# yaki-toki/5G-NR-RandomAccess

Measured on AMD Instinct MI355X. Metric: UE-subframe updates/sec at nUE=100k Beta; bit-exact success-ratio vs ref, higher is better.
Workload: dtype int32

## Files before the change

### 5g-nr-randomaccess_amd/csrc/prach_device.h

```cpp
#pragma once
#include <hip/hip_runtime.h>
#include <stdint.h>
#include "../../include/prach.h"

namespace prach {

constexpr unsigned PK_ACT_SHIFT = 0, PK_CONN_SHIFT = 2, PK_PRE_SHIFT = 4, PK_RAR_SHIFT = 12, PK_MRC_SHIFT = 20,
                   PK_PEND_SHIFT = 28;
constexpr int ACT_IDLE = 0;
constexpr int ACT_DONE = 1;
constexpr int ACT_M1 = 2;
constexpr int ACT_M3 = 3;

constexpr int PEND_NONE = 0, PEND_STAY = 1, PEND_CALLER = 2, PEND_RESET = 3, PEND_PASSIVE = 4, PEND_RJOIN = 5;
constexpr unsigned PK_GRANT_BIT = 0x80000000u;
constexpr int EV_CALLER = 1, EV_RESETCAND = 2, EV_PASSIVE = 3, EV_RJOIN = 4;

struct alignas(16) Event {
    int idx;
    int info;
    int le;
    int pad;
};

// ... 73 lines not shown
size_t trial_kernel_lds_bytes(int nP);
hipError_t launch_trial_kernel(const TrialDev *params, int ntrials, int rng_mode, int maxP, hipStream_t stream);
size_t cluster_kernel_lds_bytes(int nP, bool glibc, int lslots);
constexpr int CLUSTER_REC_G16 = 0, CLUSTER_REC_H8 = 1, CLUSTER_REC_L16 = 2;
constexpr int CLUSTER_EVW = 512;
constexpr int CLUSTER_REC_LFAST = 3;
size_t lcluster_kernel_lds_bytes(int lslots, bool glibc = false, int groups = 0);
int lcluster_group_capacity(int groups);
int lcluster_max_groups_glibc();
int lcluster_max_preambles();
hipError_t launch_lcluster_kernel(const TrialDev *params, int ntrials, int G, int lslots, int xpack, bool glibc, int groups, hipStream_t stream);
constexpr int CLUSTER_LQCAP = 4096;
constexpr size_t CLUSTER_LDS_LIMIT = 160 * 1024;
hipError_t launch_cluster_kernel(const TrialDev *params, int ntrials, int G, int maxP, int rng_mode, int rec_mode, int lslots, int xpack, hipStream_t stream);
int cluster_kernel_blocks_per_cu(int maxP, int rng_mode, int rec_mode, int lslots);
constexpr int CLUSTER_REC_BATCH = 4;
size_t batch_kernel_lds_bytes(int waves, bool glibc = false);
int batch_max_preambles();
int batch_max_rar_window();
int batch_max_subframes();
int batch_max_groups(bool glibc = false);
int batch_max_rar_window_two_per_cu();
int batch_chunk_bytes();
int batch_calendar_slots(int backoff, int accessTime, int maxRarWindow);
int batch_max_calendar_slots();
hipError_t launch_batch_kernel(const TrialDev *params, int ntrials, int waves, bool glibc, hipStream_t stream);
constexpr int STREAM_CHUNK = 31 * 2048;
hipError_t launch_glibc_stream(const unsigned *seeds, int *out, unsigned long long n, hipStream_t stream);
struct StreamJob { const unsigned *seeds; int *out; unsigned long long n; };
hipError_t launch_glibc_stream_jobs(const StreamJob *jobs, int njobs, unsigned long long max_n, hipStream_t stream);
extern "C" void prach_internal_glibc_seeds(uint32_t seed, uint64_t first, uint64_t nchunks, uint64_t chunk, uint32_t *out);
constexpr int CLUSTER_GLIBC_MAX_UE = 4096 * 64;
constexpr int CLUSTER_MAX_G = 64;
size_t noma_kernel_lds_bytes(int nP);
hipError_t launch_noma_kernel(const TrialDev *params, int ntrials, int G, int maxP, int xpack, hipStream_t stream);
int noma_kernel_blocks_per_cu(int maxP);
constexpr int NOMA_ACT_FLAG_CAP = 8192;
constexpr int NOMA_AMBIGUOUS = 77;
hipError_t launch_noma_activation(const TrialDev *params, int ntrials, int maxUE, unsigned *flags, hipStream_t stream);
constexpr int NOMA_GLIBC_AMBIGUOUS_RC = -1077;
int run_noma_glibc_trial(hipStream_t stream, const prach_cfg &c, const int32_t *hstream, unsigned long long len, prach_result *res, prach_ue_log *logs,
                         double *kernel_ms);
int run_noma_glibc_batch(hipStream_t stream, const prach_cfg *const *cfgs, int n, const unsigned long long *lens, prach_result *const *res, prach_ue_log *const *logs,
                         double *kernel_ms, int *rcs);

}
```

### 5g-nr-randomaccess_amd/csrc/prach_device_fn.h

```cpp
#pragma once
#include "prach_device.h"

#define PRACH_HD __host__ __device__ __forceinline__

namespace prach {

PRACH_HD int slot_align(int sub, int aT) {
    const int m = sub % aT;
    return m == 0 ? sub + 1 : (m == 1 ? sub : sub + (aT - m + 1));
}
struct FastMod { unsigned d, M; };
PRACH_HD unsigned mulhi32(const unsigned a, const unsigned b) { return (unsigned)(((unsigned long long)a * b) >> 32); }
PRACH_HD FastMod make_fastmod(int d) {
    FastMod f;
    f.d = (unsigned)d;
    f.M = d > 1 ? (unsigned)(0x100000000ull / (unsigned long long)d) : (d == 1 ? 0xFFFFFFFFu : 0u);
    return f;
}
PRACH_HD int fastmod(int x, const FastMod f) {
    if (f.d == 1u) return 0;
    const unsigned q = mulhi32((unsigned)x, f.M);
    const unsigned r = (unsigned)x - q * f.d;
    return (int)(r >= f.d ? r - f.d : r);
}
// ... 113 lines not shown
          n_lgain((const PRACH_G double *)d.n_lgain), n_nd0((const PRACH_G unsigned *)d.n_nd0), n_devact(d.n_devact), flags(d.flags), sector((PRACH_G int *)d.sector) {}
};

__device__ __forceinline__ int4 load_rec(const PRACH_G v4i_t *p) {
    const v4i_t v = __builtin_nontemporal_load(p);
    return make_int4(v.x, v.y, v.z, v.w);
}
__device__ __forceinline__ int4 load_rec_plain(const PRACH_G v4i_t *p) {
    const v4i_t v = *p;
    return make_int4(v.x, v.y, v.z, v.w);
}
__device__ __forceinline__ void store_rec(PRACH_G v4i_t *p, const int4 r) {
    v4i_t v;
    v.x = r.x; v.y = r.y; v.z = r.z; v.w = r.w;
    *p = v;
}
__device__ __forceinline__ void grant_rec(PRACH_G v4i_t *p) {
    __hip_atomic_fetch_or(reinterpret_cast<PRACH_G unsigned *>(p) + 3, PK_GRANT_BIT, __ATOMIC_RELAXED, __HIP_MEMORY_SCOPE_AGENT);
}
__device__ __forceinline__ void store_i2(PRACH_G v2i_t *p, const int a, const int b) {
    v2i_t v;
    v.x = a; v.y = b;
    *p = v;
}
__device__ __forceinline__ void store_log(PRACH_G v4i_t *logs, const int i, const prach_ue_log &o) {
    const int *w = reinterpret_cast<const int *>(&o);
#pragma unroll
    for (int k = 0; k < 4; k++) {
        v4i_t v;
        v.x = w[4 * k]; v.y = w[4 * k + 1]; v.z = w[4 * k + 2]; v.w = w[4 * k + 3];
        logs[(size_t)i * 4 + k] = v;
    }
}
struct PassMasks { unsigned long long light, quiet, done, trig; };
template <bool SPEC>
__device__ __forceinline__ PassMasks pass_masks(const unsigned pk, const int rx, const int rz, const int t, const unsigned rarlim, const bool front,
                                                const int i, const int acNow, const int acPrev, const int nUE) {
    typedef unsigned long long u64;
    const unsigned top = pk & 0xF0000000u;
    const u64 mM1 = __ballot((pk & 3u) == (unsigned)ACT_M1), mPre = __ballot((pk & (0xffu << PK_PRE_SHIFT)) != 0u);
    const u64 mBo = __ballot(rz <= t);
    const u64 mTrig = __ballot(rx == t);
    const u64 mPg0 = __ballot(pk < (1u << PK_PEND_SHIFT)), mAct2 = __ballot((pk & 2u) != 0u);
    u64 mDone = __ballot((pk & 3u) == (unsigned)ACT_DONE);
    const u64 mCont = mM1 & mPre & mBo;
    const unsigned age = top == ((unsigned)PEND_STAY << PK_PEND_SHIFT) ? (unsigned)(t - 1 - rx) : 0u;
    const unsigned rarnow = (pk & (0xffu << PK_RAR_SHIFT)) + (age << PK_RAR_SHIFT);
    u64 mLight = __ballot(pk < (3u << PK_PEND_SHIFT)) & mCont & __ballot(rarnow < rarlim);
    if (SPEC) mLight &= ~__ballot(top == ((unsigned)PEND_CALLER << PK_PEND_SHIFT));
    u64 mQuiet = mPg0 & (~mAct2 | (~mCont & ~mTrig & ~(mM1 & ~mPre)));
    if (front) {
        const u64 mValid = __ballot(i < acNow), mOld = __ballot(i < acPrev);
        mLight &= mOld;
        mQuiet = ~mValid | (mOld & mQuiet);
        mDone = (mValid & mDone) | __ballot(i >= nUE);
    }
    return PassMasks{mLight, mQuiet, mDone, mTrig};
}
__device__ __forceinline__ bool light_case(const unsigned pk, const int rx, const int rz, const int t, const unsigned rarlim) {
    const unsigned pg = pk >> PK_PEND_SHIFT;
    const bool contend = (pk & 3u) == (unsigned)ACT_M1 && (pk & (0xffu << PK_PRE_SHIFT)) != 0u && rz <= t;
    const int age = pg == (unsigned)PEND_STAY ? t - 1 - rx : 0;
    const unsigned rarnow = (pk & (0xffu << PK_RAR_SHIFT)) + ((unsigned)age << PK_RAR_SHIFT);
    return pg < 3u && contend && rarnow < rarlim;
}

template <class T> __device__ __forceinline__ void gadd(PRACH_G T *p, const T v) { __hip_atomic_fetch_add(p, v, __ATOMIC_RELAXED, __HIP_MEMORY_SCOPE_AGENT); }
template <class T> __device__ __forceinline__ void gmin(PRACH_G T *p, const T v) { __hip_atomic_fetch_min(p, v, __ATOMIC_RELAXED, __HIP_MEMORY_SCOPE_AGENT); }
template <class T> __device__ __forceinline__ void gmax(PRACH_G T *p, const T v) { __hip_atomic_fetch_max(p, v, __ATOMIC_RELAXED, __HIP_MEMORY_SCOPE_AGENT); }

struct UeState {
    int tx, tb, bo, act, conn, pre, rar, mrc, pend;
};
PRACH_HD UeState unpack(const int4 r) {
    UeState u;
    u.tx = r.x; u.tb = r.y; u.bo = r.z;
    u.act = (r.w >> PK_ACT_SHIFT) & 3; u.conn = (r.w >> PK_CONN_SHIFT) & 3; u.pre = (r.w >> PK_PRE_SHIFT) & 0xff;
    u.rar = (r.w >> PK_RAR_SHIFT) & 0xff; u.mrc = (r.w >> PK_MRC_SHIFT) & 0xff; u.pend = (r.w >> PK_PEND_SHIFT) & 7;
    return u;
}
PRACH_HD int4 pack(const UeState &u) {
    return make_int4(u.tx, u.tb, u.bo,
                     (u.act << PK_ACT_SHIFT) | (u.conn << PK_CONN_SHIFT) | (u.pre << PK_PRE_SHIFT) | (u.rar << PK_RAR_SHIFT) |
                         (u.mrc << PK_MRC_SHIFT) | (u.pend << PK_PEND_SHIFT));
}

}
```

### 5g-nr-randomaccess_amd/csrc/prach_engine.hip

```cpp
#include "prach_device.h"

#include <algorithm>
#include <chrono>
#include <cstdio>
#include <cstdlib>
#include <cstring>
#include <limits.h>
#include <new>
#include <thread>
#include <vector>

using namespace prach;

#define HIPCHK(expr)                                                                                  \
    do {                                                                                              \
        hipError_t e_ = (expr);                                                                       \
        if (e_ != hipSuccess) {                                                                       \
            std::fprintf(stderr, "[prach] HIP error %s at %s:%d: %s\n", hipGetErrorName(e_), __FILE__, \
                         __LINE__, hipGetErrorString(e_));                                            \
            return PRACH_ERR_DEVICE;                                                                  \
        }                                                                                             \
    } while (0)

struct prach_engine {
// ... 63 lines not shown
    evw = G == 1 ? 4096 : CLUSTER_EVW;
    const size_t lgroups = ((n + 63) / 64 + (size_t)G - 1) / (size_t)G;
    mbstride = (int)align_up((size_t)2 * (1 + c.nPreamble + evw + (lgroups + 1) / 2), 4);
    if (c.variant == PRACH_VARIANT_NOMA_C) mbstride = (int)align_up((size_t)2 * (1 + 6 * c.nPreamble), 4);
    if (G == 1) return 256;
    return 4 * (size_t)2 * G * mbstride;
}

LaunchLayout layout_launch(const prach_cfg *cfgs, const int *idx, int m, prach_ue_log *const *ue_logs, const std::vector<size_t> &stream_len, int G, bool batch, bool full_calendars, int64_t calendar_cap) {
    LaunchLayout L;
    L.t.resize(m);
    size_t o = align_up(sizeof(TrialDev) * (size_t)m, 256);
    auto take = [&](size_t bytes) { size_t at = o; o = align_up(o + bytes, 256); return at; };
    for (int k = 0; k < m; k++) {
        const prach_cfg &c = cfgs[idx[k]];
        TrialLayout &T = L.t[k];
        T.sched_len = (size_t)(prach_max_time(&c) / c.accessTime + 2);
        T.sched = take(4 * T.sched_len);
        T.stream_len = stream_len[k];
        T.nchunks = (T.stream_len + STREAM_CHUNK - 1) / STREAM_CHUNK;
        T.seeds = T.stream_len ? take(4 * 31 * (T.nchunks + 1)) : 0;
    }
    bool any_stream = false;
    for (int k = 0; k < m; k++) any_stream = any_stream || stream_len[k] > 0;
    if (any_stream) L.stream_jobs = take(sizeof(StreamJob) * (size_t)m);
    L.staged_end = o;
    L.zero_begin = o;
    L.out0 = take(sizeof(DevResult) * (size_t)m);
    for (int k = 0; k < m; k++) {
        L.t[k].out = L.out0 + sizeof(DevResult) * (size_t)k;
        const size_t mb = mbox_bytes(cfgs[idx[k]], G, L.t[k].evw, L.t[k].mbstride);
        L.t[k].mbox = mb ? take(mb) : 0;
#ifdef PRACH_STAMPS
        L.t[k].diag = G > 1 ? take(8 * 32 * (size_t)CLUSTER_MAX_G) : 0;
#else
        L.t[k].diag = 0;
#endif
    }
    if (cfgs[idx[0]].variant == PRACH_VARIANT_NOMA_C) L.act_flags = take(4 * (2 + 2 * (size_t)NOMA_ACT_FLAG_CAP));
    L.zero_end = o;
    for (int k = 0; k < m; k++) {
        const prach_cfg &c = cfgs[idx[k]];
        TrialLayout &T = L.t[k];
        const size_t n = (size_t)c.nUE;
        T.rec = T.ptc = T.ftt = T.stt = T.fcnt = T.nd = T.rec32 = T.chunks = T.ctab = T.cpool = T.jcal = T.qov = T.evov = 0;
        T.calcap = T.calslots = T.npool = T.tcap = 0;
        if (batch) {
            T.calslots = batch_calendar_slots(c.backoff, c.accessTime, c.maxRarWindow);
            const double steps_ = (double)((c.max_steps > 0 && c.max_steps < prach_max_time(&c)) ? c.max_steps : prach_max_time(&c));
            const bool overloaded = (double)c.nUE > (double)std::max(0, c.nGrantUL - 1) * steps_ / 5.0;
            T.calcap = (int)(n <= 16384 ? n : std::max<size_t>(16384, overloaded ? n * 2 / 5 : n / 8)) + 64;
            if (calendar_cap > 0) T.calcap = (int)calendar_cap;
            T.npool = 2 * (int)((n + 63) / 64) + 16 * (128 + 64) + 64;
            if (full_calendars) { T.calcap = (int)n + 64; T.npool *= 2; }
            T.tcap = (int)((n + 63) / 64) + 256;
            T.rec32 = take(32 * n); T.chunks = take((size_t)batch_chunk_bytes() * (size_t)T.npool); T.ctab = take(4 * (size_t)T.calslots * (size_t)T.tcap);
            T.cpool = take(8 * (size_t)T.npool); T.jcal = take(4 * ((size_t)T.calslots * (size_t)T.calcap + 64));
            T.qov = take(4 * n); T.evov = take(16 * n);
        } else {
            T.rec = take(16 * n);
            T.ptc = take(4 * n); T.ftt = take(4 * n); T.stt = take(4 * n); T.fcnt = take(4 * n); T.nd = take(4 * n);
        }
        T.evbuf = T.evbuf2 = T.sidx = T.cand = 0;
        if (G == 0) {
            T.evbuf = take(sizeof(Event) * n); T.evbuf2 = take(sizeof(Event) * n);
            T.sidx = take(4 * (n + 256));
        } else if (c.variant != PRACH_VARIANT_NOMA_C) {
// ... 243 lines not shown
    kc.lslots = lds_record_slots(e, cfgs, idx, m, G, maxP, &kc.maxgroups);
    kc.rec_mode = (glibc ? kc.lslots > 0 : use_fast_kernel(e, kc.lslots, maxP)) ? CLUSTER_REC_LFAST : (kc.lslots > 0 ? CLUSTER_REC_L16 : (compact ? CLUSTER_REC_H8 : CLUSTER_REC_G16));
    kc.kind = kc.rec_mode == CLUSTER_REC_LFAST ? Kernel::lcluster : Kernel::cluster;
    if (kc.rec_mode == CLUSTER_REC_H8) kc.xpack = 0;
    return kc;
}

template <class F> static void parallel_for(int nth, size_t n, const F &f) {
    nth = (int)std::min<size_t>((size_t)std::max(1, nth), std::max<size_t>(1, n));
    auto work = [&](int tix) { for (size_t j = (size_t)tix; j < n; j += (size_t)nth) f(j); };
    std::vector<std::thread> th;
    for (int tix = 1; tix < nth; tix++) th.emplace_back(work, tix);
    work(0);
    for (auto &x : th) x.join();
}

static int print_launch_diagnostics(const prach_engine *e, const prach_cfg &c, const DevResult &dr, const TrialLayout &L, const char *A, int G, bool noma) {
    if (const char *stamps = std::getenv("PRACH_PRINT_STAMPS")) {
        std::fprintf(stderr, "[prach stamps/step] pass=%.0f publish=%.0f barrier=%.0f gather=%.0f r1b=%.0f leavers=%.0f checks=%.0f grants=%.0f cycles | N avg %.1f max %llu, resetcand avg %.2f, singles avg %.1f max %llu\n",
                     dr.stamps6[0] / (double)dr.steps, dr.stamps6[1] / (double)dr.steps, dr.stamps6[2] / (double)dr.steps, dr.stamps6[3] / (double)dr.steps,
                     dr.stamps6[4] / (double)dr.steps, dr.stamps6[5] / (double)dr.steps, dr.stamps6[6] / (double)dr.steps, dr.stamps6[7] / (double)dr.steps,
                     dr.dbg[0] / (double)dr.steps, dr.dbg[1], dr.dbg[2] / (double)dr.steps, (dr.dbg[3] >> 20) / (double)dr.steps, dr.dbg[3] & 0xfffff);
        static const char *const nm[24] = {"head", "phaseB", "S1", "leavers", "S2", "publish", "window-rest", "take1", "S3", "round2", "S4", "calls", "S5", "grants", "S6", "phaseA",
                                           "w:phaseA|A-barrier", "w:loads", "w:refill", "t:buckets", "-", "-", "-", "-"};
        static const char *const nmb[24] = {"head", "joins", "-", "body", "S1", "leavers", "S2", "classify", "S4", "calls", "S5", "grants", "S6", "-", "-", "-",
                                            "-", "-", "-", "-", "-", "-", "-", "-"};
        static const char *const nmn[24] = {"head", "publish+gather", "gather-barrier", "resolve(w0)", "resolve-barrier", "passB+A(w0)", "pass-barrier", "-", "r:to-gains", "r:rank+sort", "r:pairing", "-", "-", "-", "-", "-",
                                            "-", "-", "-", "-", "-", "-", "-", "-"};
        const char *const *const names = noma ? nmn : e->last.rec_mode == CLUSTER_REC_BATCH ? nmb : nm;
        std::fprintf(stderr, "[prach fine stamps/step] nUE=%d steps=%llu", c.nUE, (unsigned long long)dr.steps);
        for (int q = 0; q < 20; q++) if (names[q][0] != '-') std::fprintf(stderr, " %s=%.0f", names[q], dr.fstamps[q] / (double)dr.steps);
        std::fprintf(stderr, "\n");
        if (L.diag && e->last.rec_mode == CLUSTER_REC_LFAST && std::atoi(stamps) >= 2) {
            std::vector<unsigned long long> dg(32 * (size_t)G);
            HIPCHK(hipMemcpy(dg.data(), A + L.diag, 8 * dg.size(), hipMemcpyDeviceToHost));
            static const char *const nmw[20] = {"head", "phaseB", "S1", "leavers", "S2", "publish", "window-rest", "take1", "S3", "round2", "S4", "calls", "S5", "grants", "S6", "-",
                                                "w:phaseA", "w:loads", "w:refill", "t:buckets"};
            for (int b_ = 0; b_ < G; b_++) {
                std::fprintf(stderr, "[prach wg stamps/step] nUE=%d steps=%llu b=%d", c.nUE, (unsigned long long)dr.steps, b_);
                for (int q = 0; q < 20; q++) if (nmw[q][0] != '-') std::fprintf(stderr, " %s=%.0f", nmw[q], dg[32 * (size_t)b_ + q] / (double)dr.steps);
                std::fprintf(stderr, " queued=%.2f late-buckets=%.3f late-header=%.3f refills=%.2f\n", dg[32 * (size_t)b_ + 24] / (double)dr.steps, dg[32 * (size_t)b_ + 25] / (double)dr.steps,
                             dg[32 * (size_t)b_ + 26] / (double)dr.steps, dg[32 * (size_t)b_ + 27] / (double)dr.steps);
            }
        }
    }
    if (dr.status != PRACH_OK && e->last.rec_mode == CLUSTER_REC_LFAST && std::getenv("PRACH_VERBOSE"))
        std::fprintf(stderr, "[prach] lcluster_kernel: trial nUE=%d left at subframe %d with status %d, capacity code %d\n", c.nUE, dr.time_exit, dr.status, dr.hard_error);
    if (dr.status == PRACH_ERR_INTERNAL && e->last.rec_mode == CLUSTER_REC_BATCH && std::getenv("PRACH_VERBOSE"))
        std::fprintf(stderr, "[prach] batch_kernel: trial nUE=%d (P %d B %d G %d R %d M %d A %d u %d) left at subframe %d: capacity %d (2 reset-cycle candidates, 3 singleton callers, 4 crossing bin, 5 a join list, 6 the grant notes, 8 a chunk table, 9 the chunk pool)\n", c.nUE, c.nPreamble, c.backoff, c.nGrantUL, c.maxRarWindow, c.maxMsg2TxCount, c.accessTime, c.uniform, dr.time_exit, dr.hard_error);
    return PRACH_OK;
}

static int run_group(prach_engine *e, CallCtx &cx, const int *idx, int m, int attempt, int G, LaunchOpts o, std::vector<int> &cal_overflow) {
    const prach_cfg *const cfgs = cx.cfgs;
    const int rng_mode = cfgs[idx[0]].rng_mode;
    const bool noma = cfgs[idx[0]].variant == PRACH_VARIANT_NOMA_C;
    std::vector<size_t> slen(m, 0);
    int maxP = 1;
    for (int k = 0; k < m; k++) {
        const prach_cfg &c = cfgs[idx[k]];
        if (rng_mode == PRACH_RNG_GLIBC) slen[k] = (size_t)stream_budget(c, attempt, e->opt_stream_factor, e->draws_per_ue_seen);
        if (c.nPreamble > maxP) maxP = c.nPreamble;
    }
    const KernelChoice kc = choose_kernel(e, cfgs, idx, m, G, maxP, o);
    const bool batch = kc.kind == Kernel::batch;
    for (int k = 0; k < m; k++)
        if ((cfgs[idx[k]].flags & PRACH_FLAG_SECTOR_GRANTS) && G > 0 && !batch) return PRACH_ERR_INTERNAL;
    const bool host_act = noma && (e->opt_noma_host_activation || o.host_act);
    const LaunchLayout LL = layout_launch(cfgs, idx, m, cx.ue_logs, slen, G, batch, o.full_calendars, e->opt_calendar_cap);
    if (LL.end > e->mem_budget && m > 1) {
        const int h = m / 2;
        int rc = run_group(e, cx, idx, h, attempt, G, o, cal_overflow);
        if (rc != PRACH_OK) return rc;
        return run_group(e, cx, idx + h, m - h, attempt, G, o, cal_overflow);
    }
// ... 545 lines not shown
```

### 5g-nr-randomaccess_amd/csrc/prach_lcluster.hip

```cpp
#include "prach_device.h"
#include "prach_device_fn.h"
#include "prach_ue_body.h"
#include "prach_exchange.h"
#include "prach_resolve.h"
#include <limits.h>

namespace prach {

namespace {

#ifdef PRACH_STAMPS
#ifndef PRACH_STAMP_TID
#define PRACH_STAMP_TID 0
#endif
#define LSTAMP(k)                                                                                      \
    do {                                                                                               \
        if (threadIdx.x == PRACH_STAMP_TID) { const unsigned long long now_ = __builtin_readcyclecounter(); fstamps[k] += now_ - fprev; fprev = now_; } \
    } while (0)
static_assert(4 * RCCAP >= 8 * 28, "diagnostic accumulators");
#else
#define LSTAMP(k) do { } while (0)
#endif

constexpr int NPCL = 64;
constexpr int NWA = NW - 1;
constexpr int LEV = 4096;
constexpr int LSC = 2048;
#ifdef PRACH_QCAP
constexpr int LCC = 8;
#else
constexpr int LCC = 1024;
#endif
constexpr int LQ = CLUSTER_LQCAP;
constexpr int LGB = 1024;
constexpr int LEPF = 32;
constexpr int LRQ = 1024;
constexpr unsigned ND_READY = 0x80000000u;

enum { S_NSUCC = 0, S_COLL, S_TXOP, S_CONTF, S_NS, S_NRC, S_NRJ, S_NEV = 8, S_NCAND , S_PTC = 13, S_FC, S_SUMT = 16,
       S_ND = 18, S_NCROSS = 20, S_NRQ = 23, S_SX = 24,
       S_QN = 26,
       S_STATUS = 28, S_NTOT = 29, S_NREM = 30, S_NSUCCTOT = 31 };

constexpr int SCHR = 32;
namespace lo {
constexpr int GEV = 0;
constexpr int SIDX = GEV + 8 * LEV;
constexpr int RCL = SIDX + 4 * LSC;
constexpr int SCAL = RCL + 4 * RCCAP;
constexpr int EVOFF = SCAL + 4 * 64;
constexpr int SCHED = SCAL + 4 * 32;
constexpr int BINS = EVOFF + 4 * 80;
constexpr int WTOT = BINS + 4 * LGB;
constexpr int PAR = WTOT + 4 * NW;
constexpr int PARSZ = 4 * 4 * NPCL;
constexpr int P_HIST = 0, P_MLOC = 4 * NPCL, P_MLOCS = 8 * NPCL, P_CANDN = 12 * NPCL;
constexpr int RB = PAR + 2 * PARSZ;
constexpr int RBSZ = 5 * 4 * NPCL;
constexpr int FCALL = RB, LCALL = RB + 4 * NPCL, TOTAL = RB + 8 * NPCL, NLV = RB + 12 * NPCL, FIE = RB + 16 * NPCL;
constexpr int QUEUE = RB + 2 * RBSZ;
constexpr int LCAND = QUEUE + 4 * LQ;
constexpr int RQ = BINS;
constexpr int TAIL = LCAND + 8 * LCC;
static_assert(LRQ <= LGB, "the refill list shares the grant bins");
static_assert(LQ <= 4 * WG_THREADS, "at most four queue batches per wavefront (the glibc mode remembers its slots in four registers)");
static_assert(SIDX % 16 == 0 && TAIL % 16 == 0 && LCAND % 8 == 0, "alignment");
}

#define LI(off) (reinterpret_cast<int *>(smem + (off)))
#define LU(off) (reinterpret_cast<unsigned *>(smem + (off)))
#define LI2(off) (reinterpret_cast<int2 *>(smem + (off)))

struct LK {
// ... 183 lines not shown
                }
            }
        }
    }
    if (GLIBC) {
        for (int g = tid; g < gcap; g += WG_THREADS) { gsum[g] = 0; gpre[g] = 0; }
        for (int x = tid; x < 4 * (lslots >> 6); x += WG_THREADS) gmask[x] = 0u;
    }
    if (tid < NPCL) {
#pragma unroll
        for (int par = 0; par < 2; par++) {
            LI(lo::PAR + par * lo::PARSZ + lo::P_HIST)[tid] = 0; LI(lo::PAR + par * lo::PARSZ + lo::P_MLOC)[tid] = INT_MAX;
            LI(lo::PAR + par * lo::PARSZ + lo::P_MLOCS)[tid] = INT_MAX; LI(lo::PAR + par * lo::PARSZ + lo::P_CANDN)[tid] = 0;
            LI(lo::FCALL + par * lo::RBSZ)[tid] = INT_MAX; LI(lo::LCALL + par * lo::RBSZ)[tid] = -1;
            LI(lo::TOTAL + par * lo::RBSZ)[tid] = 0; LI(lo::NLV + par * lo::RBSZ)[tid] = 0; LI(lo::FIE + par * lo::RBSZ)[tid] = 0;
        }
    }
    if (tid < 32) scal[tid] = 0;
    if (tid < SCHR) LI(lo::SCHED)[tid] = ((const PRACH_G int *)PD->sched)[min(tid, PD->maxTime / K.aT + 1)];
    __syncthreads();

    if (xpack && G > 1 && G <= 64) K.sx = same_xcd_handshake(mbox + parstride, mbs, b, G, &scal[S_STATUS], &scal[S_SX]);
    const bool sx = K.sx;

    int activeCheck = 0, grantCheck = 0, tlast = -1, time_exit = stop;
    unsigned long long steps = 0;
    int status = (lgroups * 64 > lslots || lslots > LQ || nP > NPCL || (GLIBC && totgroups > gcap) || G > 64 || lgroups > 64 * NWA || stop >= 0xFFFE) ? PRACH_ERR_UNSUPPORTED : PRACH_OK;
    unsigned long long deadmask = 0;
    int t5 = 0, tA = 0, slotA = 0;
    int *const ring = LI(lo::SCHED);
    const int nsched = PD->maxTime / aT + 2;
    int acNextV = ring[0];
#ifdef PRACH_STAMPS
    unsigned long long *const fstamps = reinterpret_cast<unsigned long long *>(smem + lo::RCL + 4 * (RCCAP - 56));
    unsigned long long *const dstat = fstamps + 24;
    if (tid < 28) fstamps[tid] = 0;
    unsigned long long fprev = __builtin_readcyclecounter();
#define LSTAT(k, v) do { if (threadIdx.x == PRACH_STAMP_TID) dstat[k] += (unsigned long long)(v); } while (0)
#else
#define LSTAT(k, v) do { } while (0)
#endif

    auto phase_a = [&](const bool SPEC, const int ta, const int prevA, const int acA, const int pcA) __attribute__((always_inline)) {
        int *const hist = LI(lo::PAR + pcA + lo::P_HIST), *const mloc = LI(lo::PAR + pcA + lo::P_MLOC), *const mlocs = LI(lo::PAR + pcA + lo::P_MLOCS);
        const int ngroups = (acA + 63) >> 6;
        if (w >= NWA) return;
        for (int m = 0;; m++) {
            const int j = w + NWA * m, g = b + G * j;
            if (g >= ngroups) break;
            if ((deadmask >> m) & 1ull) continue;
            const int sl = j * 64 + lane, i = g * 64 + lane;
            const int4 r = lrec[sl];
            const unsigned pk = (unsigned)r.w;
            const unsigned pg = pk >> PK_PEND_SHIFT;
            const PassMasks M = SPEC ? pass_masks<true>(pk, r.x, r.z, ta, K.rarlim, g * 64 + 64 > prevA, i, acA, prevA, nUE)
                                     : pass_masks<false>(pk, r.x, r.z, ta, K.rarlim, g * 64 + 64 > prevA, i, acA, prevA, nUE);
            const unsigned long long mHeavy = ~(M.light | M.quiet);
            if ((M.light | mHeavy) == 0ull) {
                if (M.done == ~0ull) deadmask |= 1ull << m;
                continue;
            }
            const bool lightc = __builtin_amdgcn_inverse_ballot_w64(M.light), heavy = __builtin_amdgcn_inverse_ballot_w64(mHeavy);
            const bool trig = __builtin_amdgcn_inverse_ballot_w64(M.trig);
            if (lightc) {
                const bool bump = pg != 0u;
                const bool member = bump || trig;
                if (pg != (unsigned)PEND_STAY) {
                    const unsigned npk = ((pk & 0x0FFFFFFFu) + (1u << PK_RAR_SHIFT)) | (member ? (unsigned)PEND_STAY << PK_PEND_SHIFT : 0u);
                    lrec[sl] = make_int4(bump ? ta : r.x, r.y, r.z, (int)npk);
                }
                if (member) {
                    const int p1 = (int)((pk >> PK_PRE_SHIFT) & 0xffu) - 1;
                    atomicAdd(&hist[p1], 1);
                    int *const ml = pg == (unsigned)PEND_STAY ? mlocs : mloc;
                    if (__atomic_load_n(&ml[p1], __ATOMIC_RELAXED) > i) atomicMin(&ml[p1], i);
                }
            }
            const unsigned long long hm = mHeavy;
            if (hm) {
                int base = 0;
                if (lane == 0) base = atomicAdd(&scal[S_QN + (ta & 1)], __builtin_amdgcn_readfirstlane(__popcll(hm)));
                base = __builtin_amdgcn_readlane(base, 0);
                if (heavy) queue[base + __popcll(hm & lanemask_lt(lane))] = sl;
            }
        }
    };

    auto calls = [&](const int fa_, const int N_, const bool now) __attribute__((always_inline)) {
        const int *const fcallA = LI(lo::FCALL + fa_);
        int *const lcallA = LI(lo::LCALL + fa_);
        const int nrj = now ? scal[S_NRJ] : 0;
        int my_coll = 0, my_txop = 0;
        for (int k = tid; k < N_ + nP; k += WG_THREADS) {
            int idx = 0, p = 0, ispre = 0;
            bool caller = false;
            if (k < N_) {
                const int2 e = gev[k];
                const int type = e.y & 7;
                if (type == UEV_CALLER || type == UEV_RESETCAND) { caller = true; idx = e.x; p = (e.y >> 4) & 0xff; ispre = (e.y >> 3) & 1; }
            } else {
                p = k - N_;
                if (fcallA[p] != INT_MAX && !LI(lo::FIE + fa_)[p]) { caller = true; idx = fcallA[p]; ispre = 1; }
            }
            if (!caller) continue;
            const bool first = idx == fcallA[p];
            int rj = 0;
            if (nrj > 0) {
                int prev = (!first) ? fcallA[p] : -1;
                for (int j = 0; j < N_; j++) {
                    const int2 ej = gev[j];
                    const int tj = ej.y & 7;
                    if ((tj == UEV_CALLER || tj == UEV_RESETCAND) && ((ej.y >> 4) & 0xff) == p && ej.x < idx && ej.x > prev) prev = ej.x;
                }
                for (int j = 0; j < N_; j++) {
                    const int2 ej = gev[j];
                    if ((ej.y & 7) == UEV_RJOIN && ((ej.y >> 4) & 0xff) == p && ej.x < idx && ej.x > prev) rj++;
// ... 22 lines not shown

    for (int t = 0; t < stop && status == PRACH_OK; t++) {
        int tl = tid;
        asm volatile("" : "+v"(tl));
        steps++;
        tlast = t;
        if (t5 == 0) grantCheck = 0;
        const int prevAC = activeCheck;
        if (tA == 0 && activeCheck != nUE) {
            activeCheck = __builtin_amdgcn_readfirstlane(acNextV);
            acNextV = ring[(slotA + 1) & (SCHR - 1)];
            if (slotA > 0 && (slotA & (SCHR / 2 - 1)) == 0 && tid < SCHR / 2)
                ring[(slotA + SCHR / 2 + tid) & (SCHR - 1)] = sched[min(slotA + SCHR / 2 + tid, nsched - 1)];
        }
        const int parity = t & 1;
        const unsigned tag = (unsigned)(t + 1);
        const int pc = parity * lo::PARSZ, pn = (parity ^ 1) * lo::PARSZ;
        const int fa = parity * lo::RBSZ, fb = (parity ^ 1) * lo::RBSZ;
        PRACH_G long long *const mbpar = mbox + (size_t)parity * parstride;
        PRACH_G long long *const mygr = mbpar + myoff;
        PRACH_G long long *const mbev = mygr + 1 + nP;
        int *const fcallA = LI(lo::FCALL + fa);
        const ResolveTables RT{fcallA, LI(lo::NLV + fa), LI(lo::FIE + fa), LI(lo::RCL), LI(lo::SIDX), &scal[S_NRC], &scal[S_NRJ]};
        auto ev_get = [&](const int k) __attribute__((always_inline)) { return gev[k]; };
        auto ev_kill = [&](const int k) __attribute__((always_inline)) { gev[k].y = 0; };
        LSTAMP(0);

        if (t == 0) {
            phase_a(false, 0, prevAC, activeCheck, pc);
            __syncthreads();
        }
        {
            int c_succ = 0, c_contf = 0;
            const int sl_first = queue[w * 64 + lane];
            const int qn = scal[S_QN + parity];
            LSTAT(0, qn);
            const LG GL0{nullptr, nullptr, nullptr, nullptr, 0ull};
            if (!GLIBC) {
                for (int q0 = w * 64; q0 < qn; q0 += NW * 64) {
                    const bool v = q0 + lane < qn;
                    const int sl = v ? (q0 == w * 64 ? sl_first : queue[q0 + lane]) : 0;
                    const int i = l_idx_of(K, sl);
                    int4 r = make_int4(-1, 0, 0, 0);
                    unsigned ndc = 0;
                    if (v) { r = lrec[sl]; ndc = lnd[sl]; }
                    l_step<0>(smem, K, lrec, lnd, ldraw, GL0, pc, fb, t, prevAC, mbev, tag, lane, i, sl, v && i < activeCheck, r, ndc, c_succ, c_contf);
                }
            } else {
                const unsigned long long actdraws = withnoma ? 2ull * (unsigned long long)(activeCheck - prevAC) : 0ull;
                const int ngroups_t = (activeCheck + 63) >> 6;
                const LG GC{gsum, gpre, gmask, stream, 0ull};
                for (int q0 = w * 64; q0 < qn; q0 += NW * 64) {
                    const bool v = q0 + lane < qn;
                    const int sl = v ? (q0 == w * 64 ? sl_first : queue[q0 + lane]) : 0;
                    const int i = l_idx_of(K, sl);
                    int4 r = make_int4(-1, 0, 0, 0);
                    if (v) r = lrec[sl];
                    l_step<1>(smem, K, lrec, lnd, ldraw, GC, pc, fb, t, prevAC, mbev, tag, lane, i, sl, v && i < activeCheck, r, 0u, c_succ, c_contf);
                }
                __syncthreads();
                {
                    const int nq = (lgroups + 4) / 5;
                    PRACH_G long long *const mine = mygr + 1 + nP + CLUSTER_EVW;
                    for (int q = tl; q < nq; q += WG_THREADS) {
                        unsigned c5[5];
#pragma unroll
                        for (int u_ = 0; u_ < 5; u_++) { const int g = b + G * (5 * q + u_); c5[u_] = g < totgroups ? (unsigned)gsum[g] : 0u; }
                        st_gr(sx, mine + q, mk_granule(c5[0] | (c5[1] << 8) | ((c5[2] & 0xFu) << 16), (c5[2] >> 4) | (c5[3] << 4) | (c5[4] << 12), tag));
                    }
                    for (int k = tl; k < G * nq; k += WG_THREADS) {
                        const int wg = k / nq, q = k - wg * nq;
                        if (wg == b) continue;
                        const long long g_ = wait_granule(mbpar + (unsigned)wg * mbs + 1u + (unsigned)nP + (unsigned)CLUSTER_EVW + (unsigned)q, tag, &scal[S_STATUS]);
                        const unsigned lo_ = (unsigned)g_ & 0xFFFFFu, hi_ = (unsigned)((unsigned long long)g_ >> 32) & 0xFFFFFu;
// ... 33 lines not shown
                base += tot;
            }
            if (__any((c_succ | c_contf) != 0)) {
                const int ss_ = wave_sum(c_succ), sf_ = wave_sum(c_contf);
                if (lane == 0) {
                    if (ss_) atomicAdd(&scal[S_NSUCC], ss_);
                    if (sf_) atomicAdd(&scal[S_CONTF], sf_);
                }
            }
        }
        LSTAMP(1);
        __syncthreads();
        LSTAMP(2);
        if (GLIBC) {
#pragma unroll
            for (int r_ = 0; r_ < 4; r_++) {
                if (r_ < nzs && zs[r_] >= 0) {
                    const int sl = zs[r_], jl = sl >> 6;
                    gsum[l_idx_of(K, sl) >> 6] = 0; gmask[4 * jl] = 0u; gmask[4 * jl + 1] = 0u; gmask[4 * jl + 2] = 0u; gmask[4 * jl + 3] = 0u;
                }
            }
            nzs = 0;
        }
        if (tl >= WG_THREADS - 64 && tl - (WG_THREADS - 64) < nP) {
            const int k = tl - (WG_THREADS - 64);
            const int ml = min(LI(lo::PAR + pc + lo::P_MLOC)[k], LI(lo::PAR + pc + lo::P_MLOCS)[k]);
            st_gr(sx, mygr + 1 + k, mk_granule((unsigned)LI(lo::PAR + pc + lo::P_HIST)[k], ml == INT_MAX ? GR_NONE : (unsigned)ml, tag));
        }

        {
            int *const nevp = &scal[S_NEV + 2 * parity];
            const int2 nc = *reinterpret_cast<const int2 *>(nevp);
            int nevraw = nc.x;
            if (tl == 64) { scal[S_NS] = 0; scal[S_NRC] = 0; scal[S_NRJ] = 0; scal[S_QN + parity] = 0; }
            if (nc.y > 0) {
                const int *const mloc = LI(lo::PAR + pc + lo::P_MLOC), *const mlocs = LI(lo::PAR + pc + lo::P_MLOCS);
                for (int k = tl; k < nc.y; k += WG_THREADS) {
                    const int2 c = LI2(lo::LCAND)[k];
                    if (c.x < min(mloc[c.y], mlocs[c.y])) {
                        const int es = atomicAdd(nevp, 1);
                        if (es < CLUSTER_EVW) st_gr(sx, mbev + es, mk_granule((unsigned)c.x, (unsigned)(EV_LEAVER | (c.y << 4)), tag));
                    }
                }
                LSTAMP(3);
                __syncthreads();
                LSTAMP(4);
                if (tl == 64) nevraw = *nevp;
            }
            if (tl == 64) st_gr(sx, mygr, mk_granule((unsigned)min(nevraw, CLUSTER_EVW) | ((nevraw > CLUSTER_EVW || scal[S_STATUS] == PRACH_ERR_INTERNAL) ? (1u << 13) : 0u), (unsigned)scal[S_NSUCC], tag));
        }
        LSTAMP(5);
        const bool ahead = t + 1 < stop;
        if (ahead) {
            const int acN = (tA + 1 == aT && activeCheck != nUE) ? __builtin_amdgcn_readfirstlane(acNextV) : activeCheck;
            phase_a(true, t + 1, activeCheck, acN, pn);
        }
        LSTAMP(16);
        long long gv[3] = {0, 0, 0}, hv = 0;
#pragma unroll
        for (int u = 0; u < 3; u++)
            if (r1p[u] >= 0) gv[u] = ld_sc1_64(mbpar + r1off[u]);
        if (hl >= 0 && hl < G) hv = ld_sc1_64(mbpar + hoff);
        long long ev2[2] = {0, 0};
#pragma unroll
        for (int u = 0; u < 2; u++)
            if (r2wg[u] >= 0) ev2[u] = ld_sc1_64(mbpar + r2off[u]);
        LSTAMP(17);
// ... 100 lines not shown
            if (nrc > RCCAP) { status = PRACH_ERR_INTERNAL; time_exit = t; break; }
            if (tl < 64) resolve_reset_candidates<1>(RT, nrc, nP, ev_get, ev_kill);
            else if (tl < 64 + NPCL) { LI(lo::NLV + fa)[tl - 64] = 0; LI(lo::FIE + fa)[tl - 64] = 0; }
            __syncthreads();
            for (int k = tl; k < N; k += WG_THREADS) {
                const int2 e = gev[k];
                const int type = e.y & 7, p = (e.y >> 4) & 0xff;
                if (type == EV_LEAVER) { if (e.x < fcallA[p]) atomicAdd(&LI(lo::NLV + fa)[p], 1); }
                else if ((type == UEV_CALLER || type == UEV_RESETCAND) && e.x == fcallA[p]) LI(lo::FIE + fa)[p] = 1;
            }
            __syncthreads();
        }
        const int Gr = max(0, nGrantUL - 1 - grantCheck);
        const bool defer = Gr == 0 && nrc == 0 && scal[S_NRJ] == 0 && t + 1 < stop;
        if (defer) { pendN = N; pendFa = fa; }
        else calls(fa, N, true);
        LSTAMP(11);
        if (!defer) __syncthreads();
        LSTAMP(12);
        const int ns = defer ? 0 : scal[S_NS];
        if (ns > LSC) { status = PRACH_ERR_INTERNAL; time_exit = t; break; }
        auto grant = [&](const int my) {
            const unsigned x = (unsigned)((my >> 6) - b);
            const unsigned q = x / (unsigned)G;
            const int sl = (int)(q * 64u) + (my & 63);
            atomicOr(reinterpret_cast<unsigned *>(&lrec[sl].w), PK_GRANT_BIT);
            if (ahead) {
                const int4 r = lrec[sl];
                const unsigned pk = (unsigned)r.w & ~PK_GRANT_BIT;
                if ((pk >> PK_PEND_SHIFT) == (unsigned)PEND_STAY && light_case(pk, r.x, r.z, t + 1, K.rarlim)) {
                    const int p1 = (int)((pk >> PK_PRE_SHIFT) & 0xffu) - 1;
                    atomicSub(&LI(lo::PAR + pn + lo::P_HIST)[p1], 1);
                    LI(lo::PAR + pn + lo::P_MLOCS)[p1] = INT_MAX;
                    queue[atomicAdd(&scal[S_QN + (parity ^ 1)], 1)] = sl;
                }
            }
        };
        auto mine = [&](const int my) { return ((unsigned)(my >> 6) % (unsigned)G) == (unsigned)b; };
        if (Gr > 0 && ns > 0 && ns <= 64) {
            if (tl < 64) {
                const int nsu = __builtin_amdgcn_readfirstlane(ns);
                const int my = tl < nsu ? LI(lo::SIDX)[tl] : INT_MAX;
                int rank = 0;
                for (int s_ = 0; s_ < nsu; s_++) rank += __builtin_amdgcn_readlane(my, s_) < my ? 1 : 0;
                if (tl < nsu && rank < Gr && mine(my)) grant(my);
            }
        } else if (Gr > 0 && ns > 0) {
            int *const bins = LI(lo::BINS), *const sidx = LI(lo::SIDX), *const rcl = LI(lo::RCL), *const wtot = LI(lo::WTOT);
            bins[tl] = 0;
            if (tl == 0) scal[S_NCROSS] = 0;
            __syncthreads();
            for (int j = tl; j < ns; j += WG_THREADS) atomicAdd(&bins[sidx[j] >> binshift], 1);
            __syncthreads();
            {
                const int c = bins[tl];
                const int x = wave_scan_incl(c);
                if (lane == 63) wtot[w] = x;
                __syncthreads();
                int add = 0;
                for (int k = 0; k < w; k++) add += wtot[k];
                bins[tl] = x - c + add;
            }
            __syncthreads();
            for (int j = tl; j < ns; j += WG_THREADS) {
                const int my = sidx[j];
                const int bin = my >> binshift;
                const int before = bins[bin];
// ... 54 lines not shown
                o.idx = i; o.timer = timer; o.active = u.act - 1; o.txTime = u.tx; o.firstTxTime = K.ftt[i];
                o.secondTxTime = K.stt[i]; o.nowBackoff = now_backoff(u.bo, tend); o.preamble = u.pre - 1;
                o.preambleChange = u.pre != 0; o.rarWindow = u.rar; o.maxRarCounter = u.mrc; o.preambleTxCounter = ptc;
                o.msg2Flag = (u.act == ACT_M3 || u.act == ACT_DONE); o.connectionRequest = u.conn == 2 ? 48 : u.conn;
                o.msg4Flag = u.act == ACT_DONE; o.failCount = fc;
                store_log(logs, i, o);
            }
        }
#pragma unroll
        for (int d = 32; d > 0; d >>= 1) {
            sumT += __shfl_down(sumT, d); ptcS += __shfl_down(ptcS, d); fcS += __shfl_down(fcS, d); ndS += __shfl_down(ndS, d);
        }
        if (lane == 0) {
            atomicAdd(reinterpret_cast<unsigned long long *>(&scal[S_SUMT]), (unsigned long long)sumT);
            atomicAdd(reinterpret_cast<unsigned long long *>(&scal[S_ND]), ndS);
            atomicAdd(&scal[S_PTC], ptcS);
            atomicAdd(&scal[S_FC], fcS);
        }
    }
    __syncthreads();
    if (tid == 0) {
        PRACH_G DevResult *o = (PRACH_G DevResult *)PD->out;
        gadd(&o->sumTimer, *reinterpret_cast<long long *>(&scal[S_SUMT]));
        if (GLIBC) { if (b == 0) gadd(&o->draws, base); }
        else gadd(&o->draws, *reinterpret_cast<unsigned long long *>(&scal[S_ND]));
        gadd(&o->ptcSum, scal[S_PTC]);
        gadd(&o->fcSum, scal[S_FC]);
        gadd(&o->nSuccess, scal[S_NSUCC]);
        gadd(&o->finalSuccess, scal[S_NSUCC]);
        gadd(&o->continueFailed, scal[S_CONTF]);
        if (status != PRACH_OK) gmin(&o->status, status);
        if (status == PRACH_ERR_INTERNAL) o->hard_error = 1;
#ifdef PRACH_STAMPS
        if (PD->diag) for (int k = 0; k < 28; k++) ((PRACH_G unsigned long long *)PD->diag)[b * 32 + k] = fstamps[k];
#endif
        if (b == 0) {
#ifdef PRACH_STAMPS
            for (int k = 0; k < 24; k++) o->fstamps[k] = fstamps[k];
            for (int k = 0; k < 4; k++) o->dbg[k] = dstat[k];
#endif
            o->time_exit = time_exit;
            o->collisionPreambles = scal[S_COLL];
            o->totalPreambleTxop = scal[S_TXOP];
            o->activeCheck = activeCheck;
            o->steps = steps;
        }
    }
}

size_t lcluster_kernel_lds_bytes(int lslots, bool glibc, int groups) {
    if (!glibc) return (size_t)lo::TAIL + (size_t)lslots * 28;
    return (size_t)lo::TAIL + (size_t)lslots * 16 + (size_t)lcluster_group_capacity(groups) * 8 + (size_t)(lslots / 64) * 16;
}
int lcluster_group_capacity(int groups) { return (groups + 63) / 64 * 64; }
int lcluster_max_groups_glibc() { return 4 * WG_THREADS; }
int lcluster_max_preambles() { return NPCL; }

hipError_t launch_lcluster_kernel(const TrialDev *params, int ntrials, int G, int lslots, int xpack, bool glibc, int groups, hipStream_t stream) {
    const size_t lds = lcluster_kernel_lds_bytes(lslots, glibc, groups);
    const int grid = xpack ? ((ntrials + 7) / 8) * 8 * G : ntrials * G;
    const int gcap = lcluster_group_capacity(groups);
    return launch_with_lds(glibc ? lcluster_kernel<true> : lcluster_kernel<false>, grid, WG_THREADS, lds, stream, params, G, lslots, xpack, ntrials, gcap);
}

}
```

Baseline: 19.31 billion.

## Split heavy-UE queue into front and back halves by expiry class

The heavy work queue is split in two on the non-glibc path. Expiring-candidate UEs go to the front, filled upward from one counter. All other heavy UEs, including deferred grant entries, go to the back, addressed with the index XORed by LQ-1. Even waves drain the front and odd waves drain the back, so work of the same class lands in the same wave, aiming to cut divergence in the per-UE processing loop. It also adds stamp-only diagnostics for queue classes and per-wave batch counts, at the cost of halving the waves available to each half and possibly unbalancing the load.

Result: no change. 19.18 billion (-0.7%).

```diff
diff --git a/5g-nr-randomaccess_amd/csrc/prach_device.h b/5g-nr-randomaccess_amd/csrc/prach_device.h
--- a/5g-nr-randomaccess_amd/csrc/prach_device.h
+++ b/5g-nr-randomaccess_amd/csrc/prach_device.h
@@ -129,6 +129,7 @@
 extern "C" void prach_internal_glibc_seeds(uint32_t seed, uint64_t first, uint64_t nchunks, uint64_t chunk, uint32_t *out);
 constexpr int CLUSTER_GLIBC_MAX_UE = 4096 * 64;
 constexpr int CLUSTER_MAX_G = 64;
+constexpr int LCLUSTER_DIAG_WORDS = 64;
 size_t noma_kernel_lds_bytes(int nP);
 hipError_t launch_noma_kernel(const TrialDev *params, int ntrials, int G, int maxP, int xpack, hipStream_t stream);
 int noma_kernel_blocks_per_cu(int maxP);
diff --git a/5g-nr-randomaccess_amd/csrc/prach_device_fn.h b/5g-nr-randomaccess_amd/csrc/prach_device_fn.h
--- a/5g-nr-randomaccess_amd/csrc/prach_device_fn.h
+++ b/5g-nr-randomaccess_amd/csrc/prach_device_fn.h
@@ -169,7 +169,7 @@
         logs[(size_t)i * 4 + k] = v;
     }
 }
-struct PassMasks { unsigned long long light, quiet, done, trig; };
+struct PassMasks { unsigned long long light, quiet, done, trig, expire; };
 template <bool SPEC>
 __device__ __forceinline__ PassMasks pass_masks(const unsigned pk, const int rx, const int rz, const int t, const unsigned rarlim, const bool front,
                                                 const int i, const int acNow, const int acPrev, const int nUE) {
@@ -183,16 +183,19 @@
     const u64 mCont = mM1 & mPre & mBo;
     const unsigned age = top == ((unsigned)PEND_STAY << PK_PEND_SHIFT) ? (unsigned)(t - 1 - rx) : 0u;
     const unsigned rarnow = (pk & (0xffu << PK_RAR_SHIFT)) + (age << PK_RAR_SHIFT);
-    u64 mLight = __ballot(pk < (3u << PK_PEND_SHIFT)) & mCont & __ballot(rarnow < rarlim);
-    if (SPEC) mLight &= ~__ballot(top == ((unsigned)PEND_CALLER << PK_PEND_SHIFT));
+    const u64 mOpen = __ballot(rarnow < rarlim);
+    u64 mCand = __ballot(pk < (3u << PK_PEND_SHIFT)) & mCont;
+    if (SPEC) mCand &= ~__ballot(top == ((unsigned)PEND_CALLER << PK_PEND_SHIFT));
+    u64 mLight = mCand & mOpen, mExpire = mCand & ~mOpen;
     u64 mQuiet = mPg0 & (~mAct2 | (~mCont & ~mTrig & ~(mM1 & ~mPre)));
     if (front) {
         const u64 mValid = __ballot(i < acNow), mOld = __ballot(i < acPrev);
         mLight &= mOld;
+        mExpire &= mOld;
         mQuiet = ~mValid | (mOld & mQuiet);
         mDone = (mValid & mDone) | __ballot(i >= nUE);
     }
-    return PassMasks{mLight, mQuiet, mDone, mTrig};
+    return PassMasks{mLight, mQuiet, mDone, mTrig, mExpire};
 }
 __device__ __forceinline__ bool light_case(const unsigned pk, const int rx, const int rz, const int t, const unsigned rarlim) {
     const unsigned pg = pk >> PK_PEND_SHIFT;
diff --git a/5g-nr-randomaccess_amd/csrc/prach_engine.hip b/5g-nr-randomaccess_amd/csrc/prach_engine.hip
--- a/5g-nr-randomaccess_amd/csrc/prach_engine.hip
+++ b/5g-nr-randomaccess_amd/csrc/prach_engine.hip
@@ -119,7 +119,7 @@
         const size_t mb = mbox_bytes(cfgs[idx[k]], G, L.t[k].evw, L.t[k].mbstride);
         L.t[k].mbox = mb ? take(mb) : 0;
 #ifdef PRACH_STAMPS
-        L.t[k].diag = G > 1 ? take(8 * 32 * (size_t)CLUSTER_MAX_G) : 0;
+        L.t[k].diag = G > 1 ? take(8 * (size_t)LCLUSTER_DIAG_WORDS * (size_t)CLUSTER_MAX_G) : 0;
 #else
         L.t[k].diag = 0;
 #endif
@@ -429,15 +429,20 @@
         for (int q = 0; q < 20; q++) if (names[q][0] != '-') std::fprintf(stderr, " %s=%.0f", names[q], dr.fstamps[q] / (double)dr.steps);
         std::fprintf(stderr, "\n");
         if (L.diag && e->last.rec_mode == CLUSTER_REC_LFAST && std::atoi(stamps) >= 2) {
-            std::vector<unsigned long long> dg(32 * (size_t)G);
+            constexpr size_t DW = LCLUSTER_DIAG_WORDS;
+            std::vector<unsigned long long> dg(DW * (size_t)G);
             HIPCHK(hipMemcpy(dg.data(), A + L.diag, 8 * dg.size(), hipMemcpyDeviceToHost));
             static const char *const nmw[20] = {"head", "phaseB", "S1", "leavers", "S2", "publish", "window-rest", "take1", "S3", "round2", "S4", "calls", "S5", "grants", "S6", "-",
                                                 "w:phaseA", "w:loads", "w:refill", "t:buckets"};
             for (int b_ = 0; b_ < G; b_++) {
                 std::fprintf(stderr, "[prach wg stamps/step] nUE=%d steps=%llu b=%d", c.nUE, (unsigned long long)dr.steps, b_);
-                for (int q = 0; q < 20; q++) if (nmw[q][0] != '-') std::fprintf(stderr, " %s=%.0f", nmw[q], dg[32 * (size_t)b_ + q] / (double)dr.steps);
-                std::fprintf(stderr, " queued=%.2f late-buckets=%.3f late-header=%.3f refills=%.2f\n", dg[32 * (size_t)b_ + 24] / (double)dr.steps, dg[32 * (size_t)b_ + 25] / (double)dr.steps,
-                             dg[32 * (size_t)b_ + 26] / (double)dr.steps, dg[32 * (size_t)b_ + 27] / (double)dr.steps);
+                for (int q = 0; q < 20; q++) if (nmw[q][0] != '-') std::fprintf(stderr, " %s=%.0f", nmw[q], dg[DW * (size_t)b_ + q] / (double)dr.steps);
+                std::fprintf(stderr, " queued=%.2f late-buckets=%.3f late-header=%.3f refills=%.2f", dg[DW * (size_t)b_ + 24] / (double)dr.steps, dg[DW * (size_t)b_ + 25] / (double)dr.steps,
+                             dg[DW * (size_t)b_ + 26] / (double)dr.steps, dg[DW * (size_t)b_ + 27] / (double)dr.steps);
+                std::fprintf(stderr, " q:expiry=%.2f q:deferred=%.2f q:arrival=%.2f q:msg3=%.2f batches", dg[DW * (size_t)b_ + 28] / (double)dr.steps, dg[DW * (size_t)b_ + 29] / (double)dr.steps,
+                             dg[DW * (size_t)b_ + 30] / (double)dr.steps, dg[DW * (size_t)b_ + 31] / (double)dr.steps);
+                for (int w_ = 0; w_ < NW; w_++) std::fprintf(stderr, "%c%.3f", w_ ? ',' : '=', dg[DW * (size_t)b_ + 32 + w_] / (double)dr.steps);
+                std::fprintf(stderr, "\n");
             }
         }
     }
diff --git a/5g-nr-randomaccess_amd/csrc/prach_lcluster.hip b/5g-nr-randomaccess_amd/csrc/prach_lcluster.hip
--- a/5g-nr-randomaccess_amd/csrc/prach_lcluster.hip
+++ b/5g-nr-randomaccess_amd/csrc/prach_lcluster.hip
@@ -17,7 +17,8 @@
     do {                                                                                               \
         if (threadIdx.x == PRACH_STAMP_TID) { const unsigned long long now_ = __builtin_readcyclecounter(); fstamps[k] += now_ - fprev; fprev = now_; } \
     } while (0)
-static_assert(4 * RCCAP >= 8 * 28, "diagnostic accumulators");
+constexpr int LDIAG = 24 + 8 + NW;
+static_assert(4 * RCCAP >= 8 * LDIAG, "diagnostic accumulators");
 #else
 #define LSTAMP(k) do { } while (0)
 #endif
@@ -32,13 +33,16 @@
 constexpr int LCC = 1024;
 #endif
 constexpr int LQ = CLUSTER_LQCAP;
+static_assert((LQ & (LQ - 1)) == 0, "the back end of the queue is addressed by x ^ (LQ - 1)");
 constexpr int LGB = 1024;
 constexpr int LEPF = 32;
 constexpr int LRQ = 1024;
 constexpr unsigned ND_READY = 0x80000000u;
 
 enum { S_NSUCC = 0, S_COLL, S_TXOP, S_CONTF, S_NS, S_NRC, S_NRJ, S_NEV = 8, S_NCAND , S_PTC = 13, S_FC, S_SUMT = 16,
-       S_ND = 18, S_NCROSS = 20, S_NRQ = 23, S_SX = 24,
+       S_ND = 18, S_NCROSS = 20,
+       S_QB = 21,
+       S_NRQ = 23, S_SX = 24,
        S_QN = 26,
        S_STATUS = 28, S_NTOT = 29, S_NREM = 30, S_NSUCCTOT = 31 };
 
@@ -288,13 +292,18 @@
     const int nsched = PD->maxTime / aT + 2;
     int acNextV = ring[0];
 #ifdef PRACH_STAMPS
-    unsigned long long *const fstamps = reinterpret_cast<unsigned long long *>(smem + lo::RCL + 4 * (RCCAP - 56));
+    unsigned long long *const fstamps = reinterpret_cast<unsigned long long *>(smem + lo::RCL + 4 * (RCCAP - 2 * LDIAG));
     unsigned long long *const dstat = fstamps + 24;
-    if (tid < 28) fstamps[tid] = 0;
+    unsigned long long *const wbat = dstat + 8;
+    if (tid < LDIAG) fstamps[tid] = 0;
     unsigned long long fprev = __builtin_readcyclecounter();
 #define LSTAT(k, v) do { if (threadIdx.x == PRACH_STAMP_TID) dstat[k] += (unsigned long long)(v); } while (0)
+#define LCLASS(k, m) do { if (lane == 0 && (m)) atomicAdd(&dstat[k], (unsigned long long)__popcll(m)); } while (0)
+#define LBATCH() do { if (lane == 0) wbat[w] += 1ull; } while (0)
 #else
 #define LSTAT(k, v) do { } while (0)
+#define LCLASS(k, m) do { } while (0)
+#define LBATCH() do { } while (0)
 #endif
 
     auto phase_a = [&](const bool SPEC, const int ta, const int prevA, const int acA, const int pcA) __attribute__((always_inline)) {
@@ -334,10 +343,24 @@
             }
             const unsigned long long hm = mHeavy;
             if (hm) {
+                const unsigned long long fm = GLIBC ? hm : hm & M.expire;
+#ifdef PRACH_STAMPS
+                LCLASS(4, hm & M.expire); LCLASS(5, hm & ~M.expire & __ballot(pg != 0u)); LCLASS(6, hm & ~M.expire & __ballot(pg == 0u && (pk & 2u) == 0u));
+                LCLASS(7, hm & ~M.expire & __ballot(pg == 0u && (pk & 3u) == (unsigned)ACT_M3));
+#endif
                 int base = 0;
-                if (lane == 0) base = atomicAdd(&scal[S_QN + (ta & 1)], __builtin_amdgcn_readfirstlane(__popcll(hm)));
-                base = __builtin_amdgcn_readlane(base, 0);
-                if (heavy) queue[base + __popcll(hm & lanemask_lt(lane))] = sl;
+                if (GLIBC) {
+                    if (lane == 0) base = atomicAdd(&scal[S_QN + (ta & 1)], __builtin_amdgcn_readfirstlane(__popcll(hm)));
+                    base = __builtin_amdgcn_readlane(base, 0);
+                    if (heavy) queue[base + __popcll(hm & lanemask_lt(lane))] = sl;
+                } else {
+                    const int nf = __popcll(fm);
+                    if (lane < 2) base = atomicAdd(&scal[(lane ? S_QB : S_QN) + (ta & 1)], lane ? __popcll(hm) - nf : nf);
+                    const bool fr = __builtin_amdgcn_inverse_ballot_w64(fm);
+                    auto lanes_below = [&](const unsigned long long m) __attribute__((always_inline)) { return (int)__builtin_amdgcn_mbcnt_hi((unsigned)(m >> 32), __builtin_amdgcn_mbcnt_lo((unsigned)m, 0u)); };
+                    const int belowf = lanes_below(fm), below = fr ? belowf : lanes_below(hm) - belowf;
+                    if (heavy) queue[fr ? __builtin_amdgcn_readlane(base, 0) + below : (__builtin_amdgcn_readlane(base, 1) + below) ^ (LQ - 1)] = sl;
+                }
             }
         }
     };
@@ -426,14 +449,21 @@
         }
         {
             int c_succ = 0, c_contf = 0;
-            const int sl_first = queue[w * 64 + lane];
-            const int qn = scal[S_QN + parity];
-            LSTAT(0, qn);
+            const int wb = GLIBC ? w : (w >> 1), qx = GLIBC ? 0 : -(w & 1) & (LQ - 1);
+            constexpr int QSTR = (GLIBC ? NW : NW / 2) * 64;
+            auto qslot = [&](int q) __attribute__((always_inline)) {
+                if (!GLIBC) asm volatile("" : "+v"(q));
+                return queue[q ^ qx];
+            };
+            const int sl_first = qslot(wb * 64 + lane);
+            const int qn = scal[S_QN + parity - (GLIBC ? 0 : (w & 1) * (S_QN - S_QB))];
+            LSTAT(0, scal[S_QN + parity] + scal[S_QB + parity]);
             const LG GL0{nullptr, nullptr, nullptr, nullptr, 0ull};
             if (!GLIBC) {
-                for (int q0 = w * 64; q0 < qn; q0 += NW * 64) {
+                for (int q0 = wb * 64; q0 < qn; q0 += QSTR) {
+                    LBATCH();
                     const bool v = q0 + lane < qn;
-                    const int sl = v ? (q0 == w * 64 ? sl_first : queue[q0 + lane]) : 0;
+                    const int sl = v ? (q0 == wb * 64 ? sl_first : qslot(q0 + lane)) : 0;
                     const int i = l_idx_of(K, sl);
                     int4 r = make_int4(-1, 0, 0, 0);
                     unsigned ndc = 0;
@@ -533,7 +563,7 @@
             int *const nevp = &scal[S_NEV + 2 * parity];
             const int2 nc = *reinterpret_cast<const int2 *>(nevp);
             int nevraw = nc.x;
-            if (tl == 64) { scal[S_NS] = 0; scal[S_NRC] = 0; scal[S_NRJ] = 0; scal[S_QN + parity] = 0; }
+            if (tl == 64) { scal[S_NS] = 0; scal[S_NRC] = 0; scal[S_NRJ] = 0; scal[S_QN + parity] = 0; scal[S_QB + parity] = 0; }
             if (nc.y > 0) {
                 const int *const mloc = LI(lo::PAR + pc + lo::P_MLOC), *const mlocs = LI(lo::PAR + pc + lo::P_MLOCS);
                 for (int k = tl; k < nc.y; k += WG_THREADS) {
@@ -700,7 +730,8 @@
                     const int p1 = (int)((pk >> PK_PRE_SHIFT) & 0xffu) - 1;
                     atomicSub(&LI(lo::PAR + pn + lo::P_HIST)[p1], 1);
                     LI(lo::PAR + pn + lo::P_MLOCS)[p1] = INT_MAX;
-                    queue[atomicAdd(&scal[S_QN + (parity ^ 1)], 1)] = sl;
+                    if (GLIBC) queue[atomicAdd(&scal[S_QN + (parity ^ 1)], 1)] = sl;
+                    else queue[atomicAdd(&scal[S_QB + (parity ^ 1)], 1) ^ (LQ - 1)] = sl;
                 }
             }
         };
@@ -821,7 +852,7 @@
         if (status != PRACH_OK) gmin(&o->status, status);
         if (status == PRACH_ERR_INTERNAL) o->hard_error = 1;
 #ifdef PRACH_STAMPS
-        if (PD->diag) for (int k = 0; k < 28; k++) ((PRACH_G unsigned long long *)PD->diag)[b * 32 + k] = fstamps[k];
+        if (PD->diag) for (int k = 0; k < LDIAG; k++) ((PRACH_G unsigned long long *)PD->diag)[b * LCLUSTER_DIAG_WORDS + k] = fstamps[k];
 #endif
         if (b == 0) {
 #ifdef PRACH_STAMPS
```
